# davidesantangelo/krep

Measured on NVIDIA H100. Metric: GB/s scanned (HBM-resident corpus), higher is better.
Workload: dtype u8

## Files before the change

### include/krep_b200.h

```cpp
#ifndef KREP_B200_H
#define KREP_B200_H

#include <stdbool.h>
#include <stddef.h>
#include <stdint.h>

#ifdef __cplusplus
extern "C" {
#endif

#ifndef KREP_H

typedef struct
{
   size_t start_offset;
   size_t end_offset;
} match_position_t;

typedef struct match_result_t
{
   match_position_t *positions;
   uint64_t count;
   uint64_t capacity;
} match_result_t;
// ... 65 lines not shown
bool krep_b200_ac_trie_root_has_outputs(const ac_trie_t *trie);

match_result_t *krep_b200_match_result_init(uint64_t initial_capacity);
bool krep_b200_match_result_add(match_result_t *result, size_t start_offset, size_t end_offset);
void krep_b200_match_result_free(match_result_t *result);
bool krep_b200_match_result_merge(match_result_t *dest, const match_result_t *src, size_t chunk_offset);


enum
{
   KREP_B200_ALGO_BMH = 0,
   KREP_B200_ALGO_KMP = 1,
   KREP_B200_ALGO_MEMCHR = 2,
   KREP_B200_ALGO_MEMCHR_SHORT = 3,
   KREP_B200_ALGO_SSE42 = 4,
   KREP_B200_ALGO_AVX2 = 5,
   KREP_B200_ALGO_AVX512 = 6,
   KREP_B200_ALGO_AC = 7,
   KREP_B200_ALGO_NEON = 8,
   KREP_B200_ALGO_REGEX = 9
};

typedef struct krep_b200_plan krep_b200_plan_t;

krep_b200_plan_t *krep_b200_plan_create(const search_params_t *params, int algo);
void krep_b200_plan_destroy(krep_b200_plan_t *plan);
const char *krep_b200_plan_filter_name(const krep_b200_plan_t *plan);

typedef struct
{
   const void *d_text;
   uint64_t avail_len;
   uint64_t own_begin;
   uint64_t own_end;
   uint64_t global_offset;
   int32_t prev_byte;
   int32_t next_byte;
} krep_b200_shard_t;

typedef struct
{
   uint64_t count;
   uint64_t stored;
   const uint64_t *d_keys;
   int overflow;
   uint64_t text_len;
   const uint64_t *d_line_bounds;
   int32_t device;
   int32_t slot;
   uint64_t serial;
} krep_b200_device_result_t;

int krep_b200_scan_shard(const krep_b200_plan_t *plan, const krep_b200_shard_t *shard,
                         int want_positions, void *stream, krep_b200_device_result_t *out);
int krep_b200_scan_shard_begin(const krep_b200_plan_t *plan, const krep_b200_shard_t *shard,
                               int want_positions, void *stream, int *ticket);
int krep_b200_scan_shard_end(int ticket, krep_b200_device_result_t *out);

int krep_b200_export_keys(const krep_b200_device_result_t *dev, void *d_dst, uint64_t max_keys, void *stream);
int krep_b200_export_packed(const krep_b200_device_result_t *dev, void *d_dst, uint64_t max_keys, void *stream);
int krep_b200_export_packed_async(int ticket, void *d_dst, uint64_t max_keys);
uint64_t krep_b200_merge_keys(const uint64_t *const *lists, const uint64_t *counts, uint32_t n_lists, uint64_t *dst);

float krep_b200_last_kernel_ms(void);
uint64_t krep_b200_launch_count(void);
void krep_b200_reset_launch_count(void);

typedef struct
{
   uint64_t lines;
   uint32_t flags;
   uint32_t reserved;
} krep_b200_line_count_t;
enum
{
   KREP_B200_LINES_HAS_HIT = 1,
   KREP_B200_LINES_FIRST_OPEN = 2,
   KREP_B200_LINES_LAST_PENDING = 4,
   KREP_B200_LINES_HAS_NL = 8
};
int krep_b200_count_lines_shard(const krep_b200_plan_t *plan, const search_params_t *params, const krep_b200_shard_t *shard,
                                void *stream, krep_b200_line_count_t *out);
uint64_t krep_b200_combine_line_counts(const krep_b200_line_count_t *recs, size_t n, size_t max_count);

uint64_t krep_b200_collect(const krep_b200_plan_t *plan, const search_params_t *params,
                           const krep_b200_device_result_t *dev, match_result_t *result);

uint64_t krep_b200_search_shards(const krep_b200_plan_t *plan, const search_params_t *params,
                                 const krep_b200_shard_t *shards, uint32_t n_shards, match_result_t *result);

uint64_t krep_b200_replay(int algo, const search_params_t *params, bool only_matching,
                          const uint64_t *keys, uint64_t nkeys,
                          const char *text, size_t text_len, match_result_t *result);

int64_t krep_b200_regex_filter_host(const search_params_t *params, const char *text, size_t n, uint64_t *line_starts,
                                    uint64_t cap, int *widened);

uint64_t krep_b200_replay_lines(int algo, const search_params_t *params, bool only_matching,
                                const uint64_t *keys, uint64_t nkeys, const uint64_t *bounds,
                                size_t text_len, match_result_t *result);

uint64_t krep_b200_ac_key_end(uint64_t key);
uint64_t krep_b200_ac_key_start(uint64_t key);
uint32_t krep_b200_ac_key_pattern(uint64_t key);

typedef struct
{
   uint64_t seed;
   uint64_t plant_seed;
   uint64_t plant_period;
   const char *needle;
   uint32_t needle_len;
   uint32_t flags;
} krep_b200_corpus_spec_t;

enum
{
   KREP_B200_CORPUS_RANDOM_CASE = 1,
   KREP_B200_CORPUS_EMBED_HALF = 2
};

int krep_b200_corpus_generate(const krep_b200_corpus_spec_t *spec, void *d_dst,
                              uint64_t global_offset, uint64_t len, void *stream);
int krep_b200_corpus_generate_host(const krep_b200_corpus_spec_t *spec, void *dst,
                                   uint64_t global_offset, uint64_t len);

#ifdef __cplusplus
}
#endif
#endif
```

### krep_b200/csrc/engine.cu

```cuda
#include <cub/device/device_radix_sort.cuh>
#include <algorithm>
#include <chrono>
#include <cstdarg>
#include <cstdio>
#include <cstdlib>
#include <cstring>
#include <mutex>
#include <thread>
#include "common.h"
#include "corpus.h"
#include "engine.h"

namespace kb {

static thread_local int t_err = 0;
static thread_local char t_errmsg[512] = "";

void set_error(int code, const char *fmt, ...)
{
    t_err = code;
    va_list ap;
    va_start(ap, fmt);
    vsnprintf(t_errmsg, sizeof t_errmsg, fmt, ap);
    va_end(ap);
// ... 548 lines not shown
        a.nclasses = plan->rx->nclasses;
        a.start = plan->rx->start;
        a.nl_class = plan->rx->nl_class;
        a.out = E.d_list[slot];
        a.cap = want_positions ? E.key_cap : 0;
        a.counter = slot_counter(E, slot);
        launch_regex(a, E.sm_count, stream);
        return 0;
    }
    if (plan->is_ac)
    {
        if (sh->global_offset + sh->avail_len >= (1ull << 40))
        {
            set_error(-3, "pattern-set shards must end below 2^40 bytes of global offset (key layout, csrc/common.h)");
            return -3;
        }
        AcLaunch a;
        a.text = (const uint8_t *)sh->d_text;
        a.avail_len = sh->avail_len;
        a.own_begin = sh->own_begin;
        a.own_end = own_end;
        a.global_offset = sh->global_offset;
        a.prev_byte = sh->prev_byte;
        a.next_byte = sh->next_byte;
        a.out = E.d_list[slot];
        a.cap = want_positions ? E.key_cap : 0;
        a.counter = slot_counter(E, slot);
        a.whole_word = plan->whole_word;
        a.want_positions = (uint32_t)want_positions;
        launch_ac(plan, pd->ac, a, E.sm_count, stream);
        return 0;
    }
    LitDevParams p;
    memset(&p, 0, sizeof p);
    p.text = (const uint8_t *)sh->d_text;
    p.avail_len = sh->avail_len;
    p.own_begin = sh->own_begin;
    p.own_end = own_end;
    p.global_offset = sh->global_offset;
    p.prev_byte = sh->prev_byte;
    p.next_byte = sh->next_byte;
    uint64_t total_groups;
    if (plan->filter == FILTER_ALIGNED4)
    {
        total_groups = sh->avail_len / 16;
        p.tail_start = total_groups ? total_groups * 16 - 3 : 0;
    }
    else
    {
        total_groups = sh->avail_len >= 20 ? (sh->avail_len - 20) / 16 + 1 : 0;
        p.tail_start = total_groups * 16;
    }
    p.group_begin = sh->own_begin / 16;
    p.group_end = (own_end + 2) / 16 + 1;
    if (p.group_end > total_groups) p.group_end = total_groups;
    if (p.group_begin > p.group_end) p.group_begin = p.group_end;
    p.m = plan->m;
    p.emit_len = plan->emit_len;
    for (int d = 0; d < 4; d++) p.K[d] = plan->K[d];
    p.fold = plan->fold;
    p.win_mask = plan->win_mask;
    p.mulc[0] = 1u << 24;
    p.mulc[1] = 1u << 16;
    p.mulc[2] = 1u << 8;
    p.pat_val = pd->d_pat_val;
    p.pat_mask = pd->d_pat_mask;
    p.out = E.d_list[slot];
    p.cap = want_positions ? E.key_cap : 0;
    p.counter = slot_counter(E, slot);
    p.whole_word = plan->whole_word;
    p.want_positions = (uint32_t)want_positions;
    launch_literal(plan, p, E.sm_count, stream);
    return 0;
}

int reset_counter(DevCtx &E, int slot, cudaStream_t stream)
{
    if (E.counter_clean[slot]) return 0;
    CK(cudaMemsetAsync(slot_counter(E, slot), 0, 64, stream));
    E.counter_clean[slot] = true;
    return 0;
}

static constexpr int FIN_THREADS = 512, FIN_SLICES = 16, FIN_KEYS = FIN_THREADS / FIN_SLICES, FIN_PIECE = 2048;

__global__ void __launch_bounds__(FIN_THREADS) k_finish(unsigned long long *counter, const uint64_t *__restrict__ keys, uint64_t cap,
                                                        uint64_t *d_pack, int want_sort)
{
    __shared__ uint64_t s_keys[FIN_PIECE];
    __shared__ unsigned long long s_cnt;
    if (threadIdx.x == 0) s_cnt = counter[0];
    __syncthreads();
    const unsigned long long cnt = s_cnt;
    if (blockIdx.x == 0 && threadIdx.x == 0) d_pack[0] = cnt;
    const bool sorting = want_sort && cnt != 0 && cnt <= PACK_KEYS && cnt <= cap;
    const uint32_t n = sorting ? (uint32_t)cnt : 0u;
    const uint32_t idx = blockIdx.x * FIN_KEYS + threadIdx.x / FIN_SLICES, slice = threadIdx.x % FIN_SLICES;
    if (blockIdx.x * FIN_KEYS < n)
    {
        const uint64_t mine = idx < n ? keys[idx] : ~0ull;
        uint32_t rank = 0;
        for (uint32_t base = 0; base < n; base += FIN_PIECE)
        {
            const uint32_t m = n - base < FIN_PIECE ? n - base : FIN_PIECE;
            for (uint32_t j = threadIdx.x; j < FIN_PIECE; j += FIN_THREADS) s_keys[j] = j < m ? keys[base + j] : ~0ull;
            __syncthreads();
            const uint32_t mr = (m + 63u) & ~63u;
#pragma unroll 8
            for (uint32_t j = slice; j < mr; j += FIN_SLICES) rank += s_keys[j] < mine ? 1u : 0u;
            __syncthreads();
        }
#pragma unroll
        for (int o = 1; o < FIN_SLICES; o <<= 1) rank += __shfl_xor_sync(0xffffffffu, rank, o);
        if (idx < n && slice == 0) d_pack[1 + rank] = mine;
    }
    __syncthreads();
    if (threadIdx.x == 0)
    {
        __threadfence();
        const unsigned long long done = atomicAdd(&counter[1], 1ULL);
        if (done == gridDim.x - 1)
        {
            counter[0] = 0;
            counter[1] = 0;
        }
    }
}

int finish_scan(DevCtx &E, int slot, int want_sort, cudaStream_t stream)
{
    k_finish<<<PACK_KEYS / FIN_KEYS, FIN_THREADS, 0, stream>>>(slot_counter(E, slot), E.d_list[slot], E.key_cap, E.d_pack[slot],
                                                                 (want_sort && E.d_list[slot]) ? 1 : 0);
    CK(cudaGetLastError());
    CK(cudaMemcpyAsync(E.h_pack[slot], E.d_pack[slot], (want_sort ? PACK_KEYS + 1 : 1) * sizeof(uint64_t), cudaMemcpyDeviceToHost, stream));
    CK(cudaEventRecord(E.ev_done[slot], stream));
    count_launch();
    E.counter_clean[slot] = true;
    return 0;
}

int sort_keys(DevCtx &E, int slot, uint64_t n, int end_bit, cudaStream_t stream, const uint64_t **sorted)
{
    *sorted = E.d_list[slot];
    if (n < 2) return 0;
    cub::DoubleBuffer<uint64_t> db(E.d_list[slot], E.d_alt);
    size_t need = 0;
    CK(cub::DeviceRadixSort::SortKeys(nullptr, need, db, (int64_t)n, 0, end_bit, stream));
    if (need > E.sort_tmp_bytes)
    {
        CK(cudaStreamSynchronize(stream));
        cudaFree(E.d_sort_tmp);
        E.d_sort_tmp = nullptr;
        E.sort_tmp_bytes = 0;
        CK(cudaMalloc(&E.d_sort_tmp, need));
        E.sort_tmp_bytes = need;
    }
    CK(cub::DeviceRadixSort::SortKeys(E.d_sort_tmp, need, db, (int64_t)n, 0, end_bit, stream));
    *sorted = db.Current();
    return 0;
}

static int bits_for(uint64_t v)
{
    int b = 1;
    while (b < 64 && (v >> b)) b++;
    return b;
}

int key_end_bit(const Plan *plan, uint64_t max_offset)
{
    const int shift = plan->is_ac ? AC_END_SHIFT : LIT_TAG_BITS;
    int b = bits_for(max_offset) + shift;
    return b > 64 ? 64 : b;
}

__global__ void __launch_bounds__(256) k_line_bounds(const uint8_t *__restrict__ text, uint64_t avail, uint64_t go,
                                                     const uint64_t *__restrict__ keys, uint64_t n, int is_ac, int has_prev,
                                                     int has_next, uint64_t *__restrict__ out)
{
    const uint64_t i = ((uint64_t)blockIdx.x * blockDim.x + threadIdx.x) >> 5;
    const int lane = threadIdx.x & 31;
    if (i >= n) return;
    auto start_of = [&](uint64_t key) -> uint64_t {
        if (!is_ac) return (key >> LIT_TAG_BITS) - go;
        return (key >> AC_END_SHIFT) - (1024 - ((key >> AC_LEN_SHIFT) & 1023)) - go;
    };
    const uint64_t s = start_of(keys[i]);
    const uint64_t lb = (!is_ac && i > 0) ? start_of(keys[i - 1]) : 0;
    const uint64_t ub = (!is_ac && i + 1 < n) ? start_of(keys[i + 1]) : avail;
    uint64_t ls = (!is_ac && i > 0) ? LB_SAME_AS_PREV : (has_prev ? LB_OUTSIDE_SHARD : go);
    for (uint64_t hi = s; hi > lb;)
    {
        const uint64_t w0 = hi >= lb + 128 ? hi - 128 : lb;
        int best = -1;
#pragma unroll
        for (int k = 0; k < 4; k++)
        {
            const uint64_t p = w0 + (uint64_t)lane * 4 + k;
            if (p < hi && text[p] == '\n') best = lane * 4 + k;
        }
        best = __reduce_max_sync(0xffffffffu, best);
        if (best >= 0)
        {
            ls = go + w0 + (uint64_t)best + 1;
            break;
        }
        hi = w0;
    }
    uint64_t le = (!is_ac && i + 1 < n) ? LB_SAME_AS_NEXT : (has_next ? LB_OUTSIDE_SHARD : go + avail);
    for (uint64_t lo = s; lo < ub; lo += 128)
    {
        int best = 1 << 20;
#pragma unroll
        for (int k = 3; k >= 0; k--)
// ... 480 lines not shown
```

### krep_b200/csrc/scan_count.cu

```cuda
#include <algorithm>
#include "engine.h"
#include "lit_filters.cuh"

namespace kb {

enum : uint32_t
{
    LR_HAS_HIT = 1,
    LR_FIRST_OPEN = 2,
    LR_LAST_PENDING = 4,
    LR_HAS_NL = 8
};

struct LineRec
{
    uint32_t lines, flags;
};

struct CountDev
{
    LitDevParams p;
    uint64_t own_end;
    uint32_t part_groups, n_parts;
    uint32_t exact;
    uint32_t tail;
    LineRec *recs;
};

struct PartState
{
    uint32_t lines = 0;
    bool has_hit = false, first_open = false, pending = false, seen_nl = false;
    uint64_t covered_to = 0;
};

__device__ __noinline__ unsigned verify_exact_call(const LitDevParams &p, long long cand) { return verify_exact(p, cand); }

__device__ __forceinline__ uint32_t nl_nibble(uint32_t w)
{
    const uint32_t x = w ^ 0x0A0A0A0Au;
    const uint32_t y = ~(((x & 0x7F7F7F7Fu) + 0x7F7F7F7Fu) | x | 0x7F7F7F7Fu);
    return ((y >> 7) * 0x10204080u) >> 28;
}
__device__ __forceinline__ uint32_t nl_mask16(const uint4 &v)
{
    return nl_nibble(v.x) | (nl_nibble(v.y) << 4) | (nl_nibble(v.z) << 8) | (nl_nibble(v.w) << 12);
}
__device__ __forceinline__ uint32_t range_mask16(uint64_t unit, uint64_t lo, uint64_t hi)
{
    uint32_t m = 0xFFFFu;
    if (unit < lo) m = lo - unit >= 16 ? 0u : (m & ~((1u << (uint32_t)(lo - unit)) - 1u));
    if (unit + 16 > hi) m = hi <= unit ? 0u : (m & ((1u << (uint32_t)(hi - unit)) - 1u));
    return m;
}

__device__ __noinline__ bool scan_for_newline(const LitDevParams &p, uint64_t lo, uint64_t hi)
{
    const uint32_t lane = threadIdx.x & 31;
    if (hi > p.avail_len) hi = p.avail_len;
    for (uint64_t base = lo & ~15ull; base < hi; base += 512)
    {
        const uint64_t unit = base + 16ull * lane;
        uint32_t nm = 0;
        if (unit < hi && unit + 16 > lo)
        {
            if (unit + 16 <= p.avail_len) nm = nl_mask16(__ldg(reinterpret_cast<const uint4 *>(p.text + unit)));
            else
                for (uint64_t q = unit; q < p.avail_len; q++) nm |= (p.text[q] == '\n' ? 1u : 0u) << (uint32_t)(q - unit);
            nm &= range_mask16(unit, lo, hi);
        }
        if (__any_sync(0xffffffffu, nm != 0)) return true;
    }
    return false;
}

__device__ __forceinline__ void settle(const LitDevParams &p, PartState &S, uint64_t upto)
{
    if (S.covered_to < upto && (S.pending || (!S.has_hit && !S.seen_nl)))
        if (scan_for_newline(p, S.covered_to, upto))
        {
            S.pending = false;
            S.seen_nl = true;
        }
}

__device__ __forceinline__ void account(PartState &S, uint32_t hm, uint32_t nm)
{
    const uint32_t lane = threadIdx.x & 31;
    const bool has_nl = nm != 0;
    const uint32_t fnl = has_nl ? (uint32_t)__ffs(nm) - 1 : 0, lnl = has_nl ? 31u - (uint32_t)__clz(nm) : 0;
    const bool f = has_nl && (hm & ((1u << fnl) - 1u)) != 0;
    const bool l = has_nl && ((hm >> lnl) >> 1) != 0;
    uint32_t inner = 0;
    if (__popc(nm) >= 2)
    {
        uint32_t prev = fnl, rest = nm & (nm - 1);
        while (rest)
        {
            const uint32_t nx = (uint32_t)__ffs(rest) - 1;
            if (hm & (((1u << nx) - 1u) & ~((2u << prev) - 1u))) inner++;
            prev = nx;
            rest &= rest - 1;
        }
    }
    const uint32_t A = __ballot_sync(0xffffffffu, has_nl), T = __ballot_sync(0xffffffffu, !has_nl && hm != 0);
    const uint32_t F = __ballot_sync(0xffffffffu, f), Lm = __ballot_sync(0xffffffffu, l);
    uint32_t innersum = 0;
    if (__ballot_sync(0xffffffffu, inner != 0)) innersum = __reduce_add_sync(0xffffffffu, inner);
    if (A == 0)
    {
        if (T)
        {
            if (!S.pending)
            {
                S.lines++;
                if (!S.has_hit && !S.seen_nl) S.first_open = true;
            }
            S.pending = true;
            S.has_hit = true;
        }
        return;
    }
    const uint32_t j1 = (uint32_t)__ffs(A) - 1, jr = 31u - (uint32_t)__clz(A);
    if ((T & ((1u << j1) - 1u)) || ((F >> j1) & 1u))
    {
        if (!S.pending)
        {
            S.lines++;
            if (!S.has_hit && !S.seen_nl) S.first_open = true;
        }
        S.has_hit = true;
    }
    S.pending = false;
    S.seen_nl = true;
    bool gap = false;
    if (has_nl && lane != j1)
    {
        const uint32_t below = A & ((1u << lane) - 1u);
        const uint32_t pj = 31u - (uint32_t)__clz(below);
        const uint32_t between = ((1u << lane) - 1u) & ~((2u << pj) - 1u);
        gap = ((Lm >> pj) & 1u) || (T & between) || f;
    }
    const uint32_t G = __ballot_sync(0xffffffffu, gap);
    S.lines += (uint32_t)__popc(G) + innersum;
    if (G || innersum) S.has_hit = true;
    if (((Lm >> jr) & 1u) || ((T >> jr) >> 1))
    {
        S.lines++;
        S.has_hit = true;
        S.pending = true;
    }
}

__device__ __forceinline__ uint64_t pack_state(const PartState &S)
{
    return (uint64_t)S.lines | ((uint64_t)((S.has_hit ? 1u : 0u) | (S.first_open ? 2u : 0u) | (S.pending ? 4u : 0u) | (S.seen_nl ? 8u : 0u)) << 32);
}
__device__ __forceinline__ void unpack_state(uint64_t k, PartState &S)
{
    S.lines = (uint32_t)k;
    const uint32_t f = (uint32_t)(k >> 32);
    S.has_hit = f & 1u;
    S.first_open = f & 2u;
    S.pending = f & 4u;
    S.seen_nl = f & 8u;
}
__device__ __noinline__ uint64_t account_call(uint64_t packed, uint32_t hm, uint32_t nm)
{
    PartState S;
    unpack_state(packed, S);
    account(S, hm, nm);
    return pack_state(S);
}

template <bool WINDOW>
__device__ __noinline__ uint32_t hit_mask16(const CountDev &D, uint64_t unit, const uint4 &v, uint32_t nx)
{
    const LitDevParams &p = D.p;
    const uint32_t w[5] = {v.x, v.y, v.z, v.w, nx};
    uint32_t hm = 0;
    if (WINDOW)
    {
        const uint32_t mask = p.fold & p.win_mask, k0 = p.K[0];
#pragma unroll
        for (int k = 0; k < 4; k++)
#pragma unroll
            for (int r = 0; r < 4; r++)
            {
                const uint32_t win = r == 0 ? w[k] : __funnelshift_r(w[k], w[k + 1], 8 * r);
                if ((win & mask) == k0)
                {
                    const uint64_t st = unit + 4 * k + r;
                    const bool ok = D.exact ? (st >= p.own_begin && st < p.own_end && st + p.m <= p.avail_len)
                                            : verify_exact_call(p, (long long)st) != 0;
                    if (ok) hm |= 1u << (4 * k + r);
                }
            }
    }
    else
    {
#pragma unroll
        for (int k = 0; k < 4; k++)
#pragma unroll
            for (int d = 0; d < 4; d++)
                if ((w[k] & p.fold) == p.K[d] && verify_exact_call(p, (long long)(unit + 4 * k) - d)) hm |= 1u << (4 * k);
    }
    return hm;
}

__device__ __noinline__ PartState count_tail(const CountDev &D, PartState S, uint64_t cov, uint64_t nl_lo, uint64_t nl_hi, bool window)
{
    const LitDevParams &p = D.p;
    const uint32_t lane = threadIdx.x & 31;
    if (p.avail_len < p.emit_len && cov >= nl_hi) return S;
    const uint64_t last_start = p.avail_len >= p.emit_len ? p.avail_len - p.emit_len : 0;
    uint64_t end = nl_hi > last_start + 1 ? nl_hi : last_start + 1;
    if (!window && end < cov + 1) end = cov + 1;
    for (uint64_t base = cov; base < end; base += 32)
    {
        settle(p, S, base > nl_lo ? base : nl_lo);
        const uint64_t q = base + lane;
        uint32_t hm = 0, nm = 0;
        if (q < end)
        {
            if (p.avail_len >= p.emit_len && q >= p.tail_start && q <= last_start && verify_exact(p, (long long)q)) hm = 1;
            if (!window && q == cov && p.avail_len >= p.emit_len)
                for (uint64_t s = p.tail_start; s < cov && s <= last_start; s++)
                    if (verify_exact(p, (long long)s)) hm = 1;
            if (q >= nl_lo && q < nl_hi && q < p.avail_len && p.text[q] == '\n') nm = 1;
            if (nm) hm = 0;
        }
        account(S, hm, nm);
        S.covered_to = base + 32;
    }
    return S;
}

#ifndef KREP_B200_COUNT_MINB
#define KREP_B200_COUNT_MINB 3
#endif
template <bool WINDOW, bool FOLD, bool MASKED>
__global__ void __launch_bounds__(256, KREP_B200_COUNT_MINB) k_count_lines(const __grid_constant__ CountDev D)
{
    const LitDevParams &p = D.p;
    const uint4 *__restrict__ t4 = reinterpret_cast<const uint4 *>(p.text);
    const uint32_t lane = threadIdx.x & 31;
    const uint32_t warp_global = (blockIdx.x * blockDim.x + threadIdx.x) >> 5, total_warps = (gridDim.x * blockDim.x) >> 5;
    const uint32_t k0 = p.K[0], k1 = p.K[1], k2 = p.K[2], k3 = p.K[3], fold = p.fold, mask = p.win_mask;
    const uint32_t c1 = p.mulc[0], c2 = p.mulc[1], c3 = p.mulc[2];
    for (uint32_t pi = warp_global; pi < D.n_parts; pi += total_warps)
    {
        const uint64_t ga = p.group_begin + (uint64_t)pi * D.part_groups;
        uint64_t gb = ga + D.part_groups;
        if (gb > p.group_end) gb = p.group_end;
        const bool last_part = pi + 1 == D.n_parts;
        const uint64_t nl_lo = ga * 16 > p.own_begin ? ga * 16 : p.own_begin;
        const uint64_t nl_hi = (last_part || gb * 16 > D.own_end) ? D.own_end : gb * 16;
        PartState S;
        S.covered_to = nl_lo;
        for (uint64_t g = ga; g < gb; g += 128)
        {
            uint4 v[4];
            uint32_t nx[4];
            bool ok[4];
#pragma unroll
            for (int u = 0; u < 4; u++)
            {
                const uint64_t gi = g + 32 * u + lane;
                ok[u] = gi < gb;
                v[u] = ok[u] ? ld_stream(t4 + gi) : make_uint4(0u, 0u, 0u, 0u);
                nx[u] = 0;
                if (WINDOW && ok[u] && (lane == 31 || gi + 1 >= gb)) nx[u] = __ldg(reinterpret_cast<const uint32_t *>(t4 + gi + 1));
            }
            uint32_t cand = 0;
#pragma unroll
            for (int u = 0; u < 4; u++)
            {
                bool h;
                if (WINDOW)
                {
                    const uint32_t nb = __shfl_down_sync(0xffffffffu, v[u].x, 1);
                    if (!(lane == 31 || g + 32 * u + lane + 1 >= gb)) nx[u] = nb;
                    h = hit_vec_w<FOLD, MASKED>(v[u], nx[u], fold, mask, k0, c1, c2, c3);
                }
                else
                    h = hit_vec<FOLD>(v[u], fold, k0, k1, k2, k3);
                cand |= (h && ok[u]) ? (1u << u) : 0u;
            }
            const uint32_t any = __reduce_or_sync(0xffffffffu, cand);
            if (any)
            {
                const uint64_t tile_lo = g * 16;
                settle(p, S, tile_lo > nl_lo ? tile_lo : nl_lo);
                const bool inside = tile_lo >= nl_lo && tile_lo + 2048 <= nl_hi;
                uint64_t st = pack_state(S);
#pragma unroll
                for (int u = 0; u < 4; u++)
                {
                    const uint64_t unit = tile_lo + 512ull * u + 16ull * lane;
                    uint32_t hm = 0, nm = 0;
                    if (ok[u])
                    {
                        if ((cand >> u) & 1u) hm = hit_mask16<WINDOW>(D, unit, v[u], nx[u]);
                        nm = nl_mask16(v[u]);
                        if (!inside) nm &= range_mask16(unit, nl_lo, nl_hi);
                    }
                    st = account_call(st, hm, nm);
                }
                unpack_state(st, S);
                S.covered_to = tile_lo + 2048;
            }
        }
        if (last_part && D.tail) S = count_tail(D, S, gb * 16, nl_lo, nl_hi, WINDOW);
        uint32_t flags = 0;
        if (S.has_hit)
        {
            if (S.pending && S.covered_to < nl_hi && scan_for_newline(p, S.covered_to, nl_hi)) S.pending = false;
            flags = LR_HAS_HIT | (S.first_open ? LR_FIRST_OPEN : 0u) | (S.pending ? LR_LAST_PENDING : 0u) | LR_HAS_NL;
        }
        else
        {
            const bool nl = S.seen_nl || (S.covered_to < nl_hi && scan_for_newline(p, S.covered_to, nl_hi));
            flags = nl ? LR_HAS_NL : 0u;
        }
        if (lane == 0) D.recs[pi] = LineRec{S.lines, flags};
    }
}

__host__ __device__ __forceinline__ void append_rec(uint64_t &lines, uint32_t &flags, uint64_t blines, uint32_t bflags)
{
    const bool ah = flags & LR_HAS_HIT, bh = bflags & LR_HAS_HIT;
    if (!bh)
    {
        if (ah && (bflags & LR_HAS_NL)) flags &= ~(uint32_t)LR_LAST_PENDING;
        flags |= bflags & LR_HAS_NL;
        return;
    }
    if (!ah)
    {
        const bool had_nl = flags & LR_HAS_NL;
        lines = blines;
        flags = bflags | LR_HAS_NL * had_nl;
        if (had_nl) flags &= ~(uint32_t)LR_FIRST_OPEN;
        return;
    }
    lines += blines;
    if ((flags & LR_LAST_PENDING) && (bflags & LR_FIRST_OPEN)) lines--;
    flags = LR_HAS_HIT | LR_HAS_NL | (flags & LR_FIRST_OPEN) | (bflags & LR_LAST_PENDING);
}

__global__ void __launch_bounds__(1024) k_count_finish(const LineRec *recs, uint32_t n, uint64_t *d_out, uint64_t *h_out)
{
    __shared__ uint64_t s_lines[1024];
    __shared__ uint32_t s_flags[1024];
    const uint32_t per = (n + blockDim.x - 1) / blockDim.x;
    const uint32_t a = threadIdx.x * per, b = a + per < n ? a + per : n;
    uint64_t lines = 0;
    uint32_t flags = 0;
    for (uint32_t i = a; i < b; i++) append_rec(lines, flags, recs[i].lines, recs[i].flags);
    s_lines[threadIdx.x] = lines;
    s_flags[threadIdx.x] = flags;
    __syncthreads();
    if (threadIdx.x == 0)
    {
        lines = 0;
        flags = 0;
        for (uint32_t t = 0; t < blockDim.x; t++) append_rec(lines, flags, s_lines[t], s_flags[t]);
        d_out[0] = lines;
        d_out[1] = flags;
        h_out[0] = lines;
        h_out[1] = flags;
    }
}

#define CKC(call)                                                                                  \
    do                                                                                             \
    {                                                                                              \
        cudaError_t e_ = (call);                                                                   \
        if (e_ != cudaSuccess)                                                                     \
        {                                                                                          \
            set_error(-2, "CUDA error %s at %s:%d (%s)", cudaGetErrorName(e_), __FILE__, __LINE__, \
                      cudaGetErrorString(e_));                                                     \
            return -2;                                                                             \
        }                                                                                          \
    } while (0)

bool count_lines_eligible(const Plan *plan, const search_params_t *P, int algo)
{
    if (!P->count_lines_mode || plan->is_ac || plan->is_regex || plan->emit_len != plan->m || plan->whole_word == 2) return false;
    if (plan->pattern.find('\n') != std::string::npos) return false;
    return algo == KREP_B200_ALGO_BMH || algo == KREP_B200_ALGO_KMP || algo == KREP_B200_ALGO_MEMCHR ||
           algo == KREP_B200_ALGO_MEMCHR_SHORT || algo == KREP_B200_ALGO_SSE42;
}

int ensure_line_out(DevCtx &E, uint64_t n)
{
    if (n <= E.line_out_cap) return 0;
    CKC(cudaDeviceSynchronize());
    cudaFree(E.d_line_out);
    cudaFreeHost(E.h_line_out);
    E.d_line_out = nullptr;
    E.h_line_out = nullptr;
    E.line_out_cap = 0;
    uint64_t cap = 64;
    while (cap < n) cap *= 2;
    CKC(cudaMalloc(&E.d_line_out, cap * 2 * sizeof(uint64_t)));
    CKC(cudaHostAlloc(&E.h_line_out, cap * 2 * sizeof(uint64_t), cudaHostAllocMapped | cudaHostAllocPortable));
// ... 34 lines not shown
        total_groups = sh->avail_len >= 20 ? (sh->avail_len - 20) / 16 + 1 : 0;
        p.tail_start = total_groups * 16;
    }
    p.group_begin = sh->own_begin / 16;
    p.group_end = (own_end + 2) / 16 + 1;
    D.tail = p.group_end > total_groups ? 1u : 0u;
    if (p.group_end > total_groups) p.group_end = total_groups;
    if (p.group_begin > p.group_end) p.group_begin = p.group_end;
    p.m = plan->m;
    p.emit_len = plan->emit_len;
    for (int d = 0; d < 4; d++) p.K[d] = plan->K[d];
    p.fold = plan->fold;
    p.win_mask = plan->win_mask;
    p.mulc[0] = 1u << 24;
    p.mulc[1] = 1u << 16;
    p.mulc[2] = 1u << 8;
    p.pat_val = pd->d_pat_val;
    p.pat_mask = pd->d_pat_mask;
    p.whole_word = plan->whole_word;
    D.own_end = own_end;
    {
        bool letters = true;
        for (unsigned char ch : plan->pattern) letters &= is_alpha_c(ch);
        D.exact = (window && plan->m <= 4 && plan->whole_word == 0 && (plan->case_sensitive || letters)) ? 1u : 0u;
    }
    const uint64_t groups = p.group_end - p.group_begin;
    static uint32_t part_default = 0;
    if (!part_default)
    {
        const char *v = getenv("KREP_B200_COUNT_PART_KB");
        uint32_t kb_ = v && atoi(v) > 0 ? (uint32_t)atoi(v) : 64;
        part_default = std::max<uint32_t>(128, kb_ * 64 / 128 * 128);
    }
    uint64_t part = part_default;
    const uint64_t max_parts = 1u << 18;
    if ((groups + part - 1) / part > max_parts) part = ((groups + max_parts - 1) / max_parts + 127) / 128 * 128;
    D.part_groups = (uint32_t)part;
    D.n_parts = (uint32_t)std::max<uint64_t>((groups + part - 1) / part, 1);
    if (D.n_parts > E.line_recs_cap)
    {
        CKC(cudaStreamSynchronize(stream));
        cudaFree(E.d_line_recs);
        E.d_line_recs = nullptr;
        E.line_recs_cap = 0;
        const uint64_t cap = std::max<uint64_t>(D.n_parts, 1u << 16);
        CKC(cudaMalloc(&E.d_line_recs, cap * sizeof(LineRec)));
        E.line_recs_cap = cap;
    }
    D.recs = (LineRec *)E.d_line_recs;
    const bool folded = plan->fold != 0xFFFFFFFFu, masked = plan->win_mask != 0xFFFFFFFFu;
    const uint64_t want_blocks = ((uint64_t)D.n_parts + 7) / 8;
    const unsigned grid = (unsigned)std::min<uint64_t>(want_blocks, (uint64_t)E.sm_count * KREP_B200_COUNT_MINB);
    if (!window)
    {
        if (folded) k_count_lines<false, true, false><<<grid, 256, 0, stream>>>(D);
        else k_count_lines<false, false, false><<<grid, 256, 0, stream>>>(D);
    }
    else if (folded)
    {
        if (masked) k_count_lines<true, true, true><<<grid, 256, 0, stream>>>(D);
        else k_count_lines<true, true, false><<<grid, 256, 0, stream>>>(D);
    }
    else
    {
        if (masked) k_count_lines<true, false, true><<<grid, 256, 0, stream>>>(D);
        else k_count_lines<true, false, false><<<grid, 256, 0, stream>>>(D);
    }
    CKC(cudaGetLastError());
    k_count_finish<<<1, 1024, 0, stream>>>(D.recs, D.n_parts, E.d_line_out + 2 * index, E.h_line_out + 2 * index);
    CKC(cudaGetLastError());
    count_launch(2);
    return 0;
}

uint64_t combine_line_records(const uint64_t *recs, size_t n)
{
    uint64_t lines = 0;
    uint32_t flags = 0;
    for (size_t i = 0; i < n; i++) append_rec(lines, flags, recs[2 * i], (uint32_t)recs[2 * i + 1]);
    return lines;
}

}
```

Measured before the change: 3026.

## Rework line-count kernel accounting, prefetch tiles, and replace rank sort with bitonic

The line-count kernel now prefetches the next 2048-byte tile before processing the current one. It replaces the branchy per-lane accounting with a closed-form bitmask summary computed through ballots. Candidate verification is batched over a 64-bit mask rather than going through noinline helpers, and min blocks per SM drops from 3 to 2. The finish kernel swaps an O(n^2) rank-based sort for range-bucketed per-CTA bitonic sorts in dynamic shared memory. A host reference line counter is also added; the changes trade extra registers and shared memory for fewer calls and more memory-latency overlap.

```diff
diff --git a/include/krep_b200.h b/include/krep_b200.h
--- a/include/krep_b200.h
+++ b/include/krep_b200.h
@@ -171,6 +171,7 @@
 int krep_b200_count_lines_shard(const krep_b200_plan_t *plan, const search_params_t *params, const krep_b200_shard_t *shard,
                                 void *stream, krep_b200_line_count_t *out);
 uint64_t krep_b200_combine_line_counts(const krep_b200_line_count_t *recs, size_t n, size_t max_count);
+int krep_b200_count_lines_host(const char *text, size_t n, const char *pat, size_t m, krep_b200_line_count_t *out);
 
 uint64_t krep_b200_collect(const krep_b200_plan_t *plan, const search_params_t *params,
                            const krep_b200_device_result_t *dev, match_result_t *result);
diff --git a/krep_b200/csrc/engine.cu b/krep_b200/csrc/engine.cu
--- a/krep_b200/csrc/engine.cu
+++ b/krep_b200/csrc/engine.cu
@@ -654,37 +654,83 @@
     return 0;
 }
 
-static constexpr int FIN_THREADS = 512, FIN_SLICES = 16, FIN_KEYS = FIN_THREADS / FIN_SLICES, FIN_PIECE = 2048;
+static constexpr int FIN_THREADS = 1024, FIN_CTA_BITS = 6, FIN_CTAS = 1 << FIN_CTA_BITS, FIN_SLICE_BITS = 10;
+static constexpr size_t FIN_SMEM = PACK_KEYS * sizeof(uint64_t);
 
 __global__ void __launch_bounds__(FIN_THREADS) k_finish(unsigned long long *counter, const uint64_t *__restrict__ keys, uint64_t cap,
                                                         uint64_t *d_pack, int want_sort)
 {
-    __shared__ uint64_t s_keys[FIN_PIECE];
-    __shared__ unsigned long long s_cnt;
-    if (threadIdx.x == 0) s_cnt = counter[0];
+    extern __shared__ uint64_t s_keys[];
+    __shared__ unsigned long long s_cnt, s_min, s_max;
+    __shared__ uint32_t s_m, s_below;
+    if (threadIdx.x == 0)
+    {
+        s_cnt = counter[0];
+        s_min = ~0ull;
+        s_max = 0;
+        s_m = 0;
+        s_below = 0;
+    }
     __syncthreads();
     const unsigned long long cnt = s_cnt;
     if (blockIdx.x == 0 && threadIdx.x == 0) d_pack[0] = cnt;
     const bool sorting = want_sort && cnt != 0 && cnt <= PACK_KEYS && cnt <= cap;
     const uint32_t n = sorting ? (uint32_t)cnt : 0u;
-    const uint32_t idx = blockIdx.x * FIN_KEYS + threadIdx.x / FIN_SLICES, slice = threadIdx.x % FIN_SLICES;
-    if (blockIdx.x * FIN_KEYS < n)
-    {
-        const uint64_t mine = idx < n ? keys[idx] : ~0ull;
-        uint32_t rank = 0;
-        for (uint32_t base = 0; base < n; base += FIN_PIECE)
-        {
-            const uint32_t m = n - base < FIN_PIECE ? n - base : FIN_PIECE;
-            for (uint32_t j = threadIdx.x; j < FIN_PIECE; j += FIN_THREADS) s_keys[j] = j < m ? keys[base + j] : ~0ull;
+    if (n)
+    {
+        unsigned long long lo = ~0ull, hi = 0;
+        for (uint32_t i = threadIdx.x; i < n; i += FIN_THREADS)
+        {
+            const unsigned long long k = keys[i];
+            lo = k < lo ? k : lo;
+            hi = k > hi ? k : hi;
+        }
+        atomicMin(&s_min, lo);
+        atomicMax(&s_max, hi);
+        __syncthreads();
+        const unsigned long long kmin = s_min, range = s_max - s_min;
+        const uint32_t bits = range ? 64u - (uint32_t)__clzll((long long)range) : 0u;
+        const uint32_t sh = bits > FIN_SLICE_BITS ? bits - FIN_SLICE_BITS : 0u;
+        const uint32_t per_shift = FIN_SLICE_BITS - FIN_CTA_BITS;
+        uint32_t below = 0;
+        for (uint32_t i = threadIdx.x; i < n; i += FIN_THREADS)
+        {
+            const unsigned long long k = keys[i];
+            const uint32_t slice = (uint32_t)((k - kmin) >> sh) >> per_shift;
+            if (slice < blockIdx.x) below++;
+            else if (slice == blockIdx.x) s_keys[atomicAdd(&s_m, 1u)] = k;
+        }
+        below = __reduce_add_sync(0xffffffffu, below);
+        if ((threadIdx.x & 31) == 0 && below) atomicAdd(&s_below, below);
+        __syncthreads();
+        const uint32_t m = s_m;
+        if (m)
+        {
+            uint32_t P = 2;
+            while (P < m) P <<= 1;
+            for (uint32_t i = m + threadIdx.x; i < P; i += FIN_THREADS) s_keys[i] = ~0ull;
             __syncthreads();
-            const uint32_t mr = (m + 63u) & ~63u;
-#pragma unroll 8
-            for (uint32_t j = slice; j < mr; j += FIN_SLICES) rank += s_keys[j] < mine ? 1u : 0u;
-            __syncthreads();
-        }
-#pragma unroll
-        for (int o = 1; o < FIN_SLICES; o <<= 1) rank += __shfl_xor_sync(0xffffffffu, rank, o);
-        if (idx < n && slice == 0) d_pack[1 + rank] = mine;
+            for (uint32_t k = 2; k <= P; k <<= 1)
+                for (uint32_t j = k >> 1; j > 0; j >>= 1)
+                {
+                    for (uint32_t i = threadIdx.x; i < P; i += FIN_THREADS)
+                    {
+                        const uint32_t l = i ^ j;
+                        if (l > i)
+                        {
+                            const uint64_t a = s_keys[i], b = s_keys[l];
+                            if ((a > b) == ((i & k) == 0))
+                            {
+                                s_keys[i] = b;
+                                s_keys[l] = a;
+                            }
+                        }
+                    }
+                    __syncthreads();
+                }
+            uint64_t *out = d_pack + 1 + s_below;
+            for (uint32_t i = threadIdx.x; i < m; i += FIN_THREADS) out[i] = s_keys[i];
+        }
     }
     __syncthreads();
     if (threadIdx.x == 0)
@@ -701,7 +747,13 @@
 
 int finish_scan(DevCtx &E, int slot, int want_sort, cudaStream_t stream)
 {
-    k_finish<<<PACK_KEYS / FIN_KEYS, FIN_THREADS, 0, stream>>>(slot_counter(E, slot), E.d_list[slot], E.key_cap, E.d_pack[slot],
+    static bool smem_set[MAX_DEV] = {};
+    if (!smem_set[E.device])
+    {
+        CK(cudaFuncSetAttribute(k_finish, cudaFuncAttributeMaxDynamicSharedMemorySize, (int)FIN_SMEM));
+        smem_set[E.device] = true;
+    }
+    k_finish<<<FIN_CTAS, FIN_THREADS, FIN_SMEM, stream>>>(slot_counter(E, slot), E.d_list[slot], E.key_cap, E.d_pack[slot],
                                                                  (want_sort && E.d_list[slot]) ? 1 : 0);
     CK(cudaGetLastError());
     CK(cudaMemcpyAsync(E.h_pack[slot], E.d_pack[slot], (want_sort ? PACK_KEYS + 1 : 1) * sizeof(uint64_t), cudaMemcpyDeviceToHost, stream));
diff --git a/krep_b200/csrc/scan_count.cu b/krep_b200/csrc/scan_count.cu
--- a/krep_b200/csrc/scan_count.cu
+++ b/krep_b200/csrc/scan_count.cu
@@ -34,7 +34,62 @@
     uint64_t covered_to = 0;
 };
 
-__device__ __noinline__ unsigned verify_exact_call(const LitDevParams &p, long long cand) { return verify_exact(p, cand); }
+__host__ __device__ __forceinline__ uint32_t popc32(uint32_t x)
+{
+#ifdef __CUDA_ARCH__
+    return (uint32_t)__popc(x);
+#else
+    return (uint32_t)__builtin_popcount(x);
+#endif
+}
+__host__ __device__ __forceinline__ uint32_t clz32(uint32_t x)
+{
+#ifdef __CUDA_ARCH__
+    return (uint32_t)__clz(x);
+#else
+    return x ? (uint32_t)__builtin_clz(x) : 32u;
+#endif
+}
+
+struct LaneSum
+{
+    uint32_t inner;
+    bool lead, out;
+};
+__host__ __device__ __forceinline__ LaneSum lane_summary(uint32_t hm, uint32_t nm)
+{
+    const uint32_t y = hm | nm;
+    LaneSum s;
+    s.inner = popc32((~y + (nm << 1)) & hm & 0xFFFFu);
+    s.lead = (hm & ((nm & (0u - nm)) - 1u)) != 0;
+    s.out = (hm & (0xFFFFFFFFu << (32u - clz32(nm)))) != 0;
+    return s;
+}
+__host__ __device__ __forceinline__ bool carry_in(uint32_t lane, uint32_t D, uint32_t V, bool pending)
+{
+    const uint32_t below = D & ((1u << lane) - 1u);
+    return below ? ((V >> (31u - clz32(below))) & 1u) != 0 : pending;
+}
+__host__ __device__ __forceinline__ void account_update(PartState &S, uint32_t H, uint32_t N, uint32_t V, uint32_t Ld, uint32_t sum)
+{
+    const uint32_t D = H | N;
+    if (!S.has_hit && !S.seen_nl && (Ld & D & (0u - D))) S.first_open = true;
+    S.lines += sum;
+    S.has_hit |= H != 0;
+    S.seen_nl |= N != 0;
+    if (D) S.pending = ((V >> (31u - clz32(D))) & 1u) != 0;
+}
+
+__device__ __forceinline__ void account(PartState &S, uint32_t hm, uint32_t nm)
+{
+    const uint32_t lane = threadIdx.x & 31;
+    const LaneSum s = lane_summary(hm, nm);
+    const uint32_t H = __ballot_sync(0xffffffffu, hm != 0), N = __ballot_sync(0xffffffffu, nm != 0);
+    const uint32_t V = __ballot_sync(0xffffffffu, s.out), Ld = __ballot_sync(0xffffffffu, s.lead);
+    const bool c = carry_in(lane, H | N, V, S.pending);
+    const uint32_t sum = __reduce_add_sync(0xffffffffu, s.inner + ((s.lead && !c) ? 1u : 0u));
+    account_update(S, H, N, V, Ld, sum);
+}
 
 __device__ __forceinline__ uint32_t nl_nibble(uint32_t w)
 {
@@ -54,7 +109,7 @@
     return m;
 }
 
-__device__ __noinline__ bool scan_for_newline(const LitDevParams &p, uint64_t lo, uint64_t hi)
+__device__ __forceinline__ bool scan_for_newline(const LitDevParams &p, uint64_t lo, uint64_t hi)
 {
     const uint32_t lane = threadIdx.x & 31;
     if (hi > p.avail_len) hi = p.avail_len;
@@ -84,128 +139,34 @@
         }
 }
 
-__device__ __forceinline__ void account(PartState &S, uint32_t hm, uint32_t nm)
-{
-    const uint32_t lane = threadIdx.x & 31;
-    const bool has_nl = nm != 0;
-    const uint32_t fnl = has_nl ? (uint32_t)__ffs(nm) - 1 : 0, lnl = has_nl ? 31u - (uint32_t)__clz(nm) : 0;
-    const bool f = has_nl && (hm & ((1u << fnl) - 1u)) != 0;
-    const bool l = has_nl && ((hm >> lnl) >> 1) != 0;
-    uint32_t inner = 0;
-    if (__popc(nm) >= 2)
-    {
-        uint32_t prev = fnl, rest = nm & (nm - 1);
-        while (rest)
-        {
-            const uint32_t nx = (uint32_t)__ffs(rest) - 1;
-            if (hm & (((1u << nx) - 1u) & ~((2u << prev) - 1u))) inner++;
-            prev = nx;
-            rest &= rest - 1;
-        }
-    }
-    const uint32_t A = __ballot_sync(0xffffffffu, has_nl), T = __ballot_sync(0xffffffffu, !has_nl && hm != 0);
-    const uint32_t F = __ballot_sync(0xffffffffu, f), Lm = __ballot_sync(0xffffffffu, l);
-    uint32_t innersum = 0;
-    if (__ballot_sync(0xffffffffu, inner != 0)) innersum = __reduce_add_sync(0xffffffffu, inner);
-    if (A == 0)
-    {
-        if (T)
-        {
-            if (!S.pending)
-            {
-                S.lines++;
-                if (!S.has_hit && !S.seen_nl) S.first_open = true;
-            }
-            S.pending = true;
-            S.has_hit = true;
-        }
-        return;
-    }
-    const uint32_t j1 = (uint32_t)__ffs(A) - 1, jr = 31u - (uint32_t)__clz(A);
-    if ((T & ((1u << j1) - 1u)) || ((F >> j1) & 1u))
-    {
-        if (!S.pending)
-        {
-            S.lines++;
-            if (!S.has_hit && !S.seen_nl) S.first_open = true;
-        }
-        S.has_hit = true;
-    }
-    S.pending = false;
-    S.seen_nl = true;
-    bool gap = false;
-    if (has_nl && lane != j1)
-    {
-        const uint32_t below = A & ((1u << lane) - 1u);
-        const uint32_t pj = 31u - (uint32_t)__clz(below);
-        const uint32_t between = ((1u << lane) - 1u) & ~((2u << pj) - 1u);
-        gap = ((Lm >> pj) & 1u) || (T & between) || f;
-    }
-    const uint32_t G = __ballot_sync(0xffffffffu, gap);
-    S.lines += (uint32_t)__popc(G) + innersum;
-    if (G || innersum) S.has_hit = true;
-    if (((Lm >> jr) & 1u) || ((T >> jr) >> 1))
-    {
-        S.lines++;
-        S.has_hit = true;
-        S.pending = true;
-    }
-}
-
-__device__ __forceinline__ uint64_t pack_state(const PartState &S)
-{
-    return (uint64_t)S.lines | ((uint64_t)((S.has_hit ? 1u : 0u) | (S.first_open ? 2u : 0u) | (S.pending ? 4u : 0u) | (S.seen_nl ? 8u : 0u)) << 32);
-}
-__device__ __forceinline__ void unpack_state(uint64_t k, PartState &S)
-{
-    S.lines = (uint32_t)k;
-    const uint32_t f = (uint32_t)(k >> 32);
-    S.has_hit = f & 1u;
-    S.first_open = f & 2u;
-    S.pending = f & 4u;
-    S.seen_nl = f & 8u;
-}
-__device__ __noinline__ uint64_t account_call(uint64_t packed, uint32_t hm, uint32_t nm)
-{
-    PartState S;
-    unpack_state(packed, S);
-    account(S, hm, nm);
-    return pack_state(S);
-}
-
-template <bool WINDOW>
-__device__ __noinline__ uint32_t hit_mask16(const CountDev &D, uint64_t unit, const uint4 &v, uint32_t nx)
-{
-    const LitDevParams &p = D.p;
-    const uint32_t w[5] = {v.x, v.y, v.z, v.w, nx};
-    uint32_t hm = 0;
+template <bool FOLD, bool MASKED>
+__device__ __forceinline__ uint32_t win_bits4(uint32_t lo, uint32_t hi, uint32_t mask, uint32_t k0, uint32_t c1, uint32_t c2, uint32_t c3)
+{
+    uint32_t x0 = lo, x1 = hi * c1 + __umulhi(lo, c1), x2 = hi * c2 + __umulhi(lo, c2), x3 = hi * c3 + __umulhi(lo, c3);
+    if (MASKED)
+    {
+        x0 &= mask; x1 &= mask; x2 &= mask; x3 &= mask;
+    }
+    return (x0 == k0 ? 1u : 0u) | (x1 == k0 ? 2u : 0u) | (x2 == k0 ? 4u : 0u) | (x3 == k0 ? 8u : 0u);
+}
+template <bool WINDOW, bool FOLD, bool MASKED>
+__device__ __forceinline__ uint32_t cand_mask16(const uint4 &v, uint32_t nx, uint32_t fold, uint32_t mask, uint32_t k0, uint32_t k1,
+                                                uint32_t k2, uint32_t k3, uint32_t c1, uint32_t c2, uint32_t c3)
+{
+    uint32_t w0 = v.x, w1 = v.y, w2 = v.z, w3 = v.w, w4 = nx;
+    if (FOLD)
+    {
+        w0 &= fold; w1 &= fold; w2 &= fold; w3 &= fold; w4 &= fold;
+    }
     if (WINDOW)
-    {
-        const uint32_t mask = p.fold & p.win_mask, k0 = p.K[0];
-#pragma unroll
-        for (int k = 0; k < 4; k++)
-#pragma unroll
-            for (int r = 0; r < 4; r++)
-            {
-                const uint32_t win = r == 0 ? w[k] : __funnelshift_r(w[k], w[k + 1], 8 * r);
-                if ((win & mask) == k0)
-                {
-                    const uint64_t st = unit + 4 * k + r;
-                    const bool ok = D.exact ? (st >= p.own_begin && st < p.own_end && st + p.m <= p.avail_len)
-                                            : verify_exact_call(p, (long long)st) != 0;
-                    if (ok) hm |= 1u << (4 * k + r);
-                }
-            }
-    }
-    else
-    {
-#pragma unroll
-        for (int k = 0; k < 4; k++)
-#pragma unroll
-            for (int d = 0; d < 4; d++)
-                if ((w[k] & p.fold) == p.K[d] && verify_exact_call(p, (long long)(unit + 4 * k) - d)) hm |= 1u << (4 * k);
-    }
-    return hm;
+        return win_bits4<FOLD, MASKED>(w0, w1, mask, k0, c1, c2, c3) | (win_bits4<FOLD, MASKED>(w1, w2, mask, k0, c1, c2, c3) << 4) |
+               (win_bits4<FOLD, MASKED>(w2, w3, mask, k0, c1, c2, c3) << 8) | (win_bits4<FOLD, MASKED>(w3, w4, mask, k0, c1, c2, c3) << 12);
+    const uint32_t w[4] = {w0, w1, w2, w3};
+    uint32_t c = 0;
+#pragma unroll
+    for (int k = 0; k < 4; k++)
+        c |= ((w[k] == k0 ? 1u : 0u) | (w[k] == k1 ? 2u : 0u) | (w[k] == k2 ? 4u : 0u) | (w[k] == k3 ? 8u : 0u)) << (4 * k);
+    return c;
 }
 
 __device__ __noinline__ PartState count_tail(const CountDev &D, PartState S, uint64_t cov, uint64_t nl_lo, uint64_t nl_hi, bool window)
@@ -236,8 +197,22 @@
     return S;
 }
 
+template <bool WINDOW>
+__device__ __forceinline__ void load_tile(const uint4 *__restrict__ t4, uint64_t g, uint64_t gb, uint32_t lane, uint4 (&v)[4], uint32_t (&nx)[4])
+{
+#pragma unroll
+    for (int u = 0; u < 4; u++)
+    {
+        const uint64_t gi = g + 32 * u + lane;
+        const bool ok = gi < gb;
+        v[u] = ok ? ld_stream(t4 + gi) : make_uint4(0u, 0u, 0u, 0u);
+        nx[u] = 0;
+        if (WINDOW && ok && (lane == 31 || gi + 1 >= gb)) nx[u] = __ldg(reinterpret_cast<const uint32_t *>(t4 + gi + 1));
+    }
+}
+
 #ifndef KREP_B200_COUNT_MINB
-#define KREP_B200_COUNT_MINB 3
+#define KREP_B200_COUNT_MINB 2
 #endif
 template <bool WINDOW, bool FOLD, bool MASKED>
 __global__ void __launch_bounds__(256, KREP_B200_COUNT_MINB) k_count_lines(const __grid_constant__ CountDev D)
@@ -248,6 +223,9 @@
     const uint32_t warp_global = (blockIdx.x * blockDim.x + threadIdx.x) >> 5, total_warps = (gridDim.x * blockDim.x) >> 5;
     const uint32_t k0 = p.K[0], k1 = p.K[1], k2 = p.K[2], k3 = p.K[3], fold = p.fold, mask = p.win_mask;
     const uint32_t c1 = p.mulc[0], c2 = p.mulc[1], c3 = p.mulc[2];
+    const bool exact = WINDOW && D.exact;
+    const uint64_t fit_hi = p.avail_len >= p.m ? p.avail_len - p.m + 1 : 0;
+    const uint64_t hit_hi = p.own_end < fit_hi ? p.own_end : fit_hi;
     for (uint32_t pi = warp_global; pi < D.n_parts; pi += total_warps)
     {
         const uint64_t ga = p.group_begin + (uint64_t)pi * D.part_groups;
@@ -258,24 +236,20 @@
         const uint64_t nl_hi = (last_part || gb * 16 > D.own_end) ? D.own_end : gb * 16;
         PartState S;
         S.covered_to = nl_lo;
+        uint4 v[4];
+        uint32_t nx[4];
+        load_tile<WINDOW>(t4, ga, gb, lane, v, nx);
         for (uint64_t g = ga; g < gb; g += 128)
         {
-            uint4 v[4];
-            uint32_t nx[4];
+            uint4 vn[4];
+            uint32_t nxn[4];
+            load_tile<WINDOW>(t4, g + 128, gb, lane, vn, nxn);
             bool ok[4];
+            uint32_t cand = 0;
 #pragma unroll
             for (int u = 0; u < 4; u++)
             {
-                const uint64_t gi = g + 32 * u + lane;
-                ok[u] = gi < gb;
-                v[u] = ok[u] ? ld_stream(t4 + gi) : make_uint4(0u, 0u, 0u, 0u);
-                nx[u] = 0;
-                if (WINDOW && ok[u] && (lane == 31 || gi + 1 >= gb)) nx[u] = __ldg(reinterpret_cast<const uint32_t *>(t4 + gi + 1));
-            }
-            uint32_t cand = 0;
-#pragma unroll
-            for (int u = 0; u < 4; u++)
-            {
+                ok[u] = g + 32 * u + lane < gb;
                 bool h;
                 if (WINDOW)
                 {
@@ -287,42 +261,51 @@
                     h = hit_vec<FOLD>(v[u], fold, k0, k1, k2, k3);
                 cand |= (h && ok[u]) ? (1u << u) : 0u;
             }
-            const uint32_t any = __reduce_or_sync(0xffffffffu, cand);
-            if (any)
+            if (__any_sync(0xffffffffu, cand != 0))
             {
                 const uint64_t tile_lo = g * 16;
                 settle(p, S, tile_lo > nl_lo ? tile_lo : nl_lo);
-                const bool inside = tile_lo >= nl_lo && tile_lo + 2048 <= nl_hi;
-                uint64_t st = pack_state(S);
+                const bool nl_inside = tile_lo >= nl_lo && tile_lo + 2048 <= nl_hi;
+                const bool hit_inside = tile_lo >= p.own_begin && tile_lo + 2048 <= hit_hi;
+                uint32_t hm[4], nm[4];
 #pragma unroll
                 for (int u = 0; u < 4; u++)
                 {
                     const uint64_t unit = tile_lo + 512ull * u + 16ull * lane;
-                    uint32_t hm = 0, nm = 0;
-                    if (ok[u])
+                    hm[u] = ok[u] ? cand_mask16<WINDOW, FOLD, MASKED>(v[u], nx[u], fold, mask, k0, k1, k2, k3, c1, c2, c3) : 0u;
+                    nm[u] = ok[u] ? nl_mask16(v[u]) : 0u;
+                    if (!nl_inside) nm[u] &= range_mask16(unit, nl_lo, nl_hi);
+                    if (exact && !hit_inside) hm[u] &= range_mask16(unit, p.own_begin, hit_hi);
+                }
+                if (!exact)
+                {
+                    uint64_t c64 = (uint64_t)hm[0] | ((uint64_t)hm[1] << 16) | ((uint64_t)hm[2] << 32) | ((uint64_t)hm[3] << 48), h64 = 0;
+                    while (c64)
                     {
-                        if ((cand >> u) & 1u) hm = hit_mask16<WINDOW>(D, unit, v[u], nx[u]);
-                        nm = nl_mask16(v[u]);
-                        if (!inside) nm &= range_mask16(unit, nl_lo, nl_hi);
+                        const uint32_t b = (uint32_t)__ffsll((long long)c64) - 1;
+                        c64 &= c64 - 1;
+                        const uint64_t unit = tile_lo + 512ull * (b >> 4) + 16ull * lane;
+                        const long long st = WINDOW ? (long long)(unit + (b & 15)) : (long long)(unit + (b & 12)) - (long long)(b & 3);
+                        if (verify_exact(p, st)) h64 |= 1ull << (WINDOW ? b : (b & ~3u));
                     }
-                    st = account_call(st, hm, nm);
+#pragma unroll
+                    for (int u = 0; u < 4; u++) hm[u] = (uint32_t)(h64 >> (16 * u)) & 0xFFFFu;
                 }
-                unpack_state(st, S);
+#pragma unroll
+                for (int u = 0; u < 4; u++) account(S, hm[u], nm[u]);
                 S.covered_to = tile_lo + 2048;
+            }
+#pragma unroll
+            for (int u = 0; u < 4; u++)
+            {
+                v[u] = vn[u];
+                nx[u] = nxn[u];
             }
         }
         if (last_part && D.tail) S = count_tail(D, S, gb * 16, nl_lo, nl_hi, WINDOW);
-        uint32_t flags = 0;
-        if (S.has_hit)
-        {
-            if (S.pending && S.covered_to < nl_hi && scan_for_newline(p, S.covered_to, nl_hi)) S.pending = false;
-            flags = LR_HAS_HIT | (S.first_open ? LR_FIRST_OPEN : 0u) | (S.pending ? LR_LAST_PENDING : 0u) | LR_HAS_NL;
-        }
-        else
-        {
-            const bool nl = S.seen_nl || (S.covered_to < nl_hi && scan_for_newline(p, S.covered_to, nl_hi));
-            flags = nl ? LR_HAS_NL : 0u;
-        }
+        settle(p, S, nl_hi);
+        const uint32_t flags = S.has_hit ? (LR_HAS_HIT | (S.first_open ? LR_FIRST_OPEN : 0u) | (S.pending ? LR_LAST_PENDING : 0u) | LR_HAS_NL)
+                                         : (S.seen_nl ? LR_HAS_NL : 0u);
         if (lane == 0) D.recs[pi] = LineRec{S.lines, flags};
     }
 }
@@ -523,3 +506,40 @@
 }
 
 }
+
+extern "C" int krep_b200_count_lines_host(const char *text, size_t n, const char *pat, size_t m, krep_b200_line_count_t *out)
+{
+    using namespace kb;
+    if (!out || (!text && n) || !pat || m == 0) return -1;
+    PartState S;
+    for (size_t base = 0; base < n; base += 512)
+    {
+        uint32_t hm[32], nm[32], H = 0, N = 0, V = 0, Ld = 0;
+        LaneSum s[32];
+        for (uint32_t lane = 0; lane < 32; lane++)
+        {
+            hm[lane] = nm[lane] = 0;
+            for (uint32_t b = 0; b < 16; b++)
+            {
+                const size_t q = base + 16 * lane + b;
+                if (q >= n) break;
+                if (text[q] == '\n') nm[lane] |= 1u << b;
+                else if (q + m <= n && memcmp(text + q, pat, m) == 0) hm[lane] |= 1u << b;
+            }
+            s[lane] = lane_summary(hm[lane], nm[lane]);
+            H |= (hm[lane] != 0 ? 1u : 0u) << lane;
+            N |= (nm[lane] != 0 ? 1u : 0u) << lane;
+            V |= (s[lane].out ? 1u : 0u) << lane;
+            Ld |= (s[lane].lead ? 1u : 0u) << lane;
+        }
+        uint32_t sum = 0;
+        for (uint32_t lane = 0; lane < 32; lane++)
+            sum += s[lane].inner + ((s[lane].lead && !carry_in(lane, H | N, V, S.pending)) ? 1u : 0u);
+        account_update(S, H, N, V, Ld, sum);
+    }
+    out->lines = S.lines;
+    out->flags = S.has_hit ? (LR_HAS_HIT | (S.first_open ? LR_FIRST_OPEN : 0u) | (S.pending ? LR_LAST_PENDING : 0u) | LR_HAS_NL)
+                           : (S.seen_nl ? LR_HAS_NL : 0u);
+    out->reserved = 0;
+    return 0;
+}
```

New measurement: 3051 (median of 6 runs). No clear change (+0.8%).
